# MathThyMod/GP_emu_UQSA

Measured on AMD Instinct MI355X. Metric: log-marginal-likelihood evals/sec at n=16384 d=10 fp64; 1/2/4/8 GPU, higher is better.
Workload: dtype f64

## Files before the change

gp_emu_uqsa_amd/csrc/gpemu.hip:

```cpp
#include <hip/hip_runtime.h>

#include <algorithm>
#include <array>
#include <atomic>
#include <map>
#include <cmath>
#include <cstdio>
#include <cstdlib>
#include <cstring>
#include <limits>
#include <string>
#include <vector>

#include "../../include/gpemu.h"
#include "gpemu_kernels.hpp"
#include "gpemu_gemm_sched.hpp"
#include "gpemu_small.hpp"
#include "gpemu_tiny.hpp"
#include "gpemu_snb.hpp"
#include "gpemu_ozaki.hpp"
#include "gpemu_pivchol.hpp"
#include "gpemu_imse.hpp"
#include "gpemu_postgrad.hpp"
#include "gpemu_postmean.hpp"
// ... 13 lines not shown
enum AdhocSlot {
  ADHOC_POST_V = ADHOC_DESC_BASE + 0,
  ADHOC_COV = ADHOC_DESC_BASE + 1,
  ADHOC_NOISE = ADHOC_DESC_BASE + 3,
  ADHOC_PIVCHOL = ADHOC_DESC_BASE + 4,
  ADHOC_POST_U = ADHOC_DESC_BASE + 5,
  ADHOC_IMSE = ADHOC_DESC_BASE + 7,
  ADHOC_TEST = ADHOC_DESC_BASE + 8,
  ADHOC_BENCH = ADHOC_DESC_BASE + 16,
};

struct Plan {
  long long n_pad = 0;
  const double* a_ptr = nullptr;
  const double* b_ptr = nullptr;
  std::vector<int> fused, fused_aug;
  std::vector<int> trtri;
  std::vector<std::vector<std::array<int, 3>>> tri_pairs;
  int lauum = -1;
  bool aug = false;
  std::vector<int> grp, grp_aug;
  int split_h = 0, aug_mid = -1;
  std::vector<int> sfused, sfused_aug, sgrp, sgrp_aug;
  bool sides = false;
  std::vector<std::array<int, 4>> trtri_side;
  std::vector<GemmLaunch> launches;
  std::vector<GemmProb> probs;
  std::vector<unsigned> tiles;
};

constexpr int FACT_FLAG_INTS = 6;

constexpr int OZ_CHOL_MIN = 8192;


struct Fact {
  long long n_pad = 0;
  int NB = 0;
  double* A = nullptr;
  double* B = nullptr;
  size_t cap = 0;
  double* logdet = nullptr;
  int* flags = nullptr;
  int* tflags = nullptr;
  bool aug = false;
  double* Faug = nullptr;
  double* part = nullptr;
  int* tcnt = nullptr;
  bool xdone[2] = {false, false};
  int xh = 0;
  int x11 = 0;
  bool t_ahead = false;
  void xclear(int h = 0) { xdone[0] = xdone[1] = t_ahead = false; x11 = 0; xh = h; }
  int desc_base = 0;
  Plan plan;
};
// ... 53 lines not shown
  double onel_tag = 0.0;
  int oz_on = 1, oz_nmod = OZ_MAXMOD;
  int oz_min_np = 6144;
  int oz_np2 = 0, oz_list_len = 0;
  long long oz_npad = 0;
  OzConst oz_c{};
  int8_t* dozp = nullptr;
  int8_t* dozr = nullptr;
  int* dozx = nullptr;
  unsigned* dozl = nullptr;
  double* dozt = nullptr;
  hipEvent_t ev_oz = nullptr;
  std::vector<OzTriPair> oz_tri;
  int oz_tri_min = 8192;
  double oz_lauum_ops = 0.0;
  int oz_chol = 1, oz_chol_min = OZ_CHOL_MIN;
  int tri_ahead_on = 1;
  hipEvent_t ev_l11 = nullptr, ev_schur = nullptr;
  OzTriPair oz_chol_q{};
  long long oz_chol_loff = 0;
  int oz_chol_llen = 0;
  double oz_chol_ops = 0.0;
  bool oz_chol_ready = false;
  bool oz_l21_valid = false;
  std::vector<hipEvent_t> oev;
  size_t oev_used = 0;
  double oz_ms = 0.0, oz_launches = 0.0, oz_ops = 0.0, oz_flops64 = 0.0;
  int dbg_skip_wait = -1;
  size_t small_cap = 0;

  double* hpin = nullptr;
  size_t hpin_cap = 0;

  float* dX32 = nullptr;
  size_t x32_cap = 0;
  bool x32_valid = false;
  float* dK32 = nullptr;
  size_t k32_cap = 0;
  hipEvent_t ev_pipe[2] = {nullptr, nullptr};
  int8_t* dpxp = nullptr;
  int* dpxe = nullptr;
  int8_t* dpkp = nullptr;
  int* dpke = nullptr;
  int8_t* dpres = nullptr;
  unsigned* dpl = nullptr;
  size_t pxp_cap = 0, pxe_cap = 0, pkp_cap = 0, pke_cap = 0, pres_cap = 0, pl_cap = 0;
// ... 237 lines not shown
  }
  return GPE_OK;
}

void add_launch(Plan& pl, GemmKind kind, const std::vector<GemmProb>& probs, double flops,
                const std::vector<unsigned>* order = nullptr) {
  GemmLaunch L = begin_launch(kind, pl.probs, flops);
  bool listable = probs.size() < 256;
  for (const GemmProb& p : probs) {
    push_prob(L, pl.probs, p, true);
    listable = listable && p.mt <= 4096 && p.nt <= 4096 && p.ksplit <= 1;
  }
  if (order) {
    set_list(L, pl.tiles, *order);
  } else if (listable) {
    const std::vector<unsigned> tl = order_tiles(probs);
    if ((int)tl.size() == L.tiles) set_list(L, pl.tiles, tl);
  }
  pl.launches.push_back(L);
}

bool oz_use(const gpe_ctx* c);
int oz_chol_split(const gpe_ctx* c, const Fact& F);

std::atomic<int> g_inflight[64];

struct InflightGuard {
  int dev;
  explicit InflightGuard(int d) : dev(d & 63) { g_inflight[dev].fetch_add(1); }
  ~InflightGuard() { g_inflight[dev].fetch_sub(1); }
};

struct AdhocGemm { GemmKind kind; GemmProb p; };
int adhoc_gemm(gpe_ctx* c, AdhocSlot slot, const std::vector<AdhocGemm>& g, GemmLaunch* out = nullptr,
               bool standalone = false) {
  std::vector<GemmProb> d;
  std::vector<GemmLaunch> launches;
  for (const AdhocGemm& e : g) {
    GemmLaunch L = begin_launch(e.kind, d);
    push_prob(L, d, e.p, standalone);
    L.first += slot;
    launches.push_back(L);
  }
  if (standalone)
    HIPCHK(c, hipMemcpy(c->dprobs + slot, d.data(), d.size() * sizeof(GemmProb), hipMemcpyHostToDevice));
  else
// ... 424 lines not shown
        for (const GemmProb& q : wb) { tb += prob_tiles(q); kb = std::max(kb, q.K); }
        for (int sd = 0; sd < 2; ++sd) {
          std::vector<GemmProb> pa, pb;
          double fa = 0.0, fb = 0.0;
          for (const auto& pr : trtri_side_pairs(pl.tri_pairs[lv], h, sd)) tri_pair(pr, pa, pb, fa, fb);
          if (pa.empty()) continue;
          split_k(pa, F.part, F.tcnt, ta, ka);
          split_k(pb, F.part, F.tcnt, tb, kb);
          side[2 * sd] = (int)pl.launches.size();
          add_launch(pl, GEMM_AK, pa, fa);
          side[2 * sd + 1] = (int)pl.launches.size();
          add_launch(pl, GEMM_PLAIN, pb, fb);
        }
        pl.trtri_side.push_back(side);
      }
      pl.sides = true;
      if ((int)pl.probs.size() > limit) {
        pl.launches.resize(nl1);
        pl.probs.resize(np1);
        pl.tiles.resize(nt1);
        pl.sides = false;
      }
    }
  }
  if ((int)pl.probs.size() > limit) return fail(c, GPE_ERR_UNSUPPORTED, "GEMM schedule too large");
  for (auto& L : pl.launches) L.first += F.desc_base;
  HIPCHK(c, hipMemcpy(c->dprobs + F.desc_base, pl.probs.data(), pl.probs.size() * sizeof(GemmProb),
                      hipMemcpyHostToDevice));
  const size_t half = pl.tiles.size() + 1;
  const size_t need = 2 * half;
  const bool regrow = need > c->tiles_cap;
  CHK(grow_buf(c, &c->dtiles, &c->tiles_cap, need));
  if (regrow) {
    Fact& other = (&F == &c->tr) ? c->aux : c->tr;
    other.plan = Plan();
  }
  const size_t base = (F.desc_base == 0) ? 0 : c->tiles_cap / 2;
  if (pl.tiles.size() > c->tiles_cap / 2) return fail(c, GPE_ERR_STATE, "tile list overflow");
  for (auto& L : pl.launches)
    if (L.list >= 0) L.list += (long long)base;
  if (!pl.tiles.empty())
    HIPCHK(c, hipMemcpy(c->dtiles + base, pl.tiles.data(), pl.tiles.size() * sizeof(unsigned),
                        hipMemcpyHostToDevice));
  return GPE_OK;
}

// ... 54 lines not shown
  if (kernel_alt(kernel)) {
    *coff = 1.0;
    *cdiag = predict ? 1.0 + nu * nu : 1.0;
  } else {
    *coff = 1.0 - nu;
    *cdiag = predict ? 1.0 : 1.0 - nu;
  }
}

int kbuild(gpe_ctx* c, int kernel, double nu, double s2, double rscale) {
  PairArgs a;
  a.xr = c->dXw; a.xc = c->dXw; a.out = c->tr.A; a.ld = c->n_pad;
  a.d = c->d; a.nr_valid = (int)c->n; a.nc_valid = (int)c->n;
  a.mt = c->NB; a.nt = c->NB; a.mode = 1 | 2;
  double coff, cdiag;
  kernel_consts(kernel, nu, true, &coff, &cdiag);
  a.s2 = s2; a.coff = coff; a.cdiag = cdiag;
  a.rscale = rscale; a.r = (c->has_r && rscale != 0.0) ? c->dr : nullptr;
  a.fam = kernel_fam(kernel);
  return launch_pairs(c, a, c->NB * (c->NB + 1) / 2);
}

int oz_prepare(gpe_ctx* c, Fact& F);
int chol_schur(gpe_ctx* c, Fact& F, hipStream_t st, bool with_aug);
int trtri(gpe_ctx* c, Fact& F, bool ozaki = false, bool ahead = false);

int potrf(gpe_ctx* c, Fact& F, bool with_aug = false, bool split = false, bool ahead = false) {
  CHK(build_plan(c, F));
  const int hs = split ? F.plan.split_h : 0;
  if (hs) CHK(oz_prepare(c, F));
  const Plan& pl = F.plan;
  if (hs != (split ? pl.split_h : 0)) return fail(c, GPE_ERR_STATE, "internal error: split plan changed");
  const int NB = F.NB;
  HIPCHK(c, hipMemsetAsync(F.flags, 0, FACT_FLAG_INTS * (size_t)NB * sizeof(int), c->stream));
  const bool wa = with_aug && pl.aug;
  const bool tri_ahead = hs && ahead && pl.sides && c->tri_ahead_on && c->chol_prio;
  F.xclear(tri_ahead ? hs : 0);
  const bool grp = c->potrf_group &&
                   (c->potrf_mode == 1 || (c->potrf_mode == 0 && g_inflight[c->device & 63].load() <= 1));
  const std::vector<int>& fidx = hs ? (grp ? (wa ? pl.sgrp_aug : pl.sgrp) : (wa ? pl.sfused_aug : pl.sfused))
                                    : (grp ? (wa ? pl.grp_aug : pl.grp) : (wa ? pl.fused_aug : pl.fused));
  if (c->chol_prio) {
    HIPCHK(c, hipEventRecord(c->ev_fork, c->stream));
    HIPCHK(c, hipStreamWaitEvent(c->stream2, c->ev_fork, 0));
    for (int t = 0; t < NB; ++t) {
      if (hs && t == hs) {
        if (tri_ahead) HIPCHK(c, hipEventRecord(c->ev_l11, c->stream2));
        CHK(chol_schur(c, F, c->stream2, wa));
        if (tri_ahead) {
          HIPCHK(c, hipEventRecord(c->ev_schur, c->stream2));
          CHK(trtri(c, F, true, true));
        }
      }
      if (fidx[t] >= 0) CHK(launch_gemm_range(c, pl.launches[fidx[t]], c->stream2));
    }
    HIPCHK(c, hipEventRecord(c->ev_join, c->stream2));
    HIPCHK(c, hipStreamWaitEvent(c->stream, c->ev_join, 0));
    return GPE_OK;
  }
#ifdef GEMM_TTRACE
  if (const char* es = std::getenv("GPEMU_DEBUG_STOP_STEP")) {
    const int stop = std::atoi(es);
    for (int t = 0; t <= stop && t < NB; ++t)
      if (fidx[t] >= 0) CHK(launch_gemm_range(c, pl.launches[fidx[t]]));
    HIPCHK(c, hipStreamSynchronize(c->stream));
    return fail(c, GPE_ERR_STATE, "debug stop after Cholesky launch " + std::to_string(stop));
  }
#endif
  for (int t = 0; t < NB; ++t) {
    if (hs && t == hs) CHK(chol_schur(c, F, c->stream, wa));
    if (fidx[t] >= 0) CHK(launch_gemm_range(c, pl.launches[fidx[t]]));
  }
  return GPE_OK;
}

void ev_rec(gpe_ctx* c, int i);

int lauum(gpe_ctx* c, Fact& F) {
  CHK(build_plan(c, F));
  return launch_gemm_range(c, F.plan.launches[F.plan.lauum]);
}

int ensure_xdiag(gpe_ctx* c, Fact& F, int side = -1) {
  const bool want0 = side != 1 && !F.xdone[0], want1 = side != 0 && !F.xdone[1];
  const int a = want0 ? 0 : F.xh, b = want1 ? F.NB : F.xh;
  if (b > a) {
    const long long off = (long long)a * TILE * (F.n_pad + 1);
    hipLaunchKernelGGL(k_xasm, dim3(b - a), dim3(256), DB_LDS_DOUBLES * sizeof(double), c->stream, F.A + off, F.B + off,
                       (long long)F.n_pad);
    HIPCHK(c, hipGetLastError());
  }
  F.xdone[0] = F.xdone[0] || want0;
  F.xdone[1] = F.xdone[1] || want1;
// ... 206 lines not shown
int z_from_factor(gpe_ctx* c);
int trsv_lower(gpe_ctx* c, Fact& F, const double* R, long long ldr, int P, double* Y, long long ldy);

int factor_and_invert(gpe_ctx* c, int kernel, const double* delta, double nu, double s2,
                      double rscale, bool invert = true, bool objective = false) {
  c->linv_valid = false;
  c->oz_l21_valid = false;
  HIPCHK(c, hipStreamSynchronize(c->stream2));
  HIPCHK(c, hipMemsetAsync(c->dinfo, 0, sizeof(int), c->stream));
  CHK(build_plan(c, c->tr));
  ev_rec(c, 0);
  CHK(scale_training(c, delta));
  CHK(kbuild(c, kernel, nu, s2, rscale));
  const int P = c->q + 1;
  c->zaug_valid = !invert && c->tr.plan.aug && P <= TILE;
  if (c->zaug_valid) {
    const long long tot = c->n_pad * TILE;
    hipLaunchKernelGGL(k_aug_init, dim3((unsigned)((tot + 255) / 256)), dim3(256), 0, c->stream, c->dF,
                       c->n_pad, P, c->n_pad, c->tr.Faug);
    HIPCHK(c, hipGetLastError());
  }
  ev_rec(c, 1);
  CHK(build_plan(c, c->tr));
  CHK(potrf(c, c->tr, c->zaug_valid, objective && (invert || c->oz_chol >= 2), objective && invert));
  if (kernel_fam(kernel) != FAM_GAUSS) {
    double coff, cdiag;
    kernel_consts(kernel, nu, true, &coff, &cdiag);
    const double floor_rel = 4.0 * (double)c->n_pad * std::numeric_limits<double>::epsilon();
    const double* r = (c->has_r && rscale != 0.0) ? c->dr : nullptr;
    hipLaunchKernelGGL(k_pivot_floor, dim3((unsigned)((c->n + 255) / 256)), dim3(256), 0, c->stream, c->tr.A,
                       c->n_pad, (int)c->n, floor_rel, s2 * cdiag, r, rscale, c->dinfo);
    HIPCHK(c, hipGetLastError());
  }
  ev_rec(c, 2);
  if (invert) {
    CHK(trtri(c, c->tr, true));
    c->linv_valid = true;
  }
  CHK(z_from_factor(c));
  ev_rec(c, 3);
  return GPE_OK;
}

int z_from_factor(gpe_ctx* c) {
  const int P = c->q + 1;
  const long long np = c->n_pad;
  if (c->zaug_valid) {
// ... 20 lines not shown
  CHK(ensure_xdiag(c, F));
  for (int c0 = 0; c0 < P; c0 += TS_PM) {
    const int pc = std::min(TS_PM, P - c0);
    HIPCHK(c, hipMemsetAsync(F.tflags, 0, 2 * sizeof(int), c->stream));
    hipLaunchKernelGGL(k_trsv_lower, dim3(F.NB), dim3(512), 0, c->stream, F.A, (long long)F.n_pad, F.B,
                       R + (long long)c0 * ldr, ldr, Y + (long long)c0 * ldy, ldy, pc, F.tflags, F.tflags + 1,
                       c->dinfo);
    HIPCHK(c, hipGetLastError());
  }
  return GPE_OK;
}

constexpr int OZ_MIN_NP = 6144, OZ_POST_MIN_NP = 4096, OZ_MAX_NP = 65536, OZ_POST_MAX_NP = 32768;
static_assert(OZ_MAX_NP % OZ_T == 0 && OZ_MAX_NP <= OZ_MAX_K && OZ_POST_MAX_NP <= OZ_MAX_K, "int8 sums too long");
bool oz_use(const gpe_ctx* c) { return c->oz_on && c->n_pad >= c->oz_min_np && c->n_pad <= OZ_MAX_NP; }

int oz_chol_split(const gpe_ctx* c, const Fact& F) {
  if (!c->oz_chol || !oz_use(c) || F.n_pad != c->n_pad || F.NB < 2) return 0;
  int h = 1;
  while (2 * h < F.NB) h *= 2;
  return (F.NB - h) * TILE >= c->oz_chol_min ? h : 0;
}

bool oz_tri_level(const gpe_ctx* c, const std::vector<std::array<int, 3>>& prs) {
  return oz_use(c) && !prs.empty() && (prs[0][1] - prs[0][0]) * TILE >= c->oz_tri_min;
}

int oz_prepare(gpe_ctx* c, Fact& F) {
  const int np2 = (int)(((c->n_pad + OZ_T - 1) / OZ_T) * OZ_T);
  if (c->n_pad == c->oz_npad && np2 == c->oz_np2 && c->oz_c.nmod == c->oz_nmod) return GPE_OK;
  c->oz_np2 = 0;
  c->oz_npad = 0;
  c->oz_chol_ready = false;
  c->oz_l21_valid = false;
  CHK(build_plan(c, F));
  const int N = c->oz_nmod;
  size_t planes = (size_t)oz_plane_bytes(np2) * N;
  size_t resid = (size_t)oz_lauum_shape(np2).res_bytes() * N;
  size_t scratch = 0, nex = (size_t)np2;
  std::vector<unsigned> all = oz_lauum_shape(np2).list();
  c->oz_list_len = (int)all.size();
  c->oz_lauum_ops = oz_lauum_shape(np2).ops(N);
  c->oz_tri.clear();
  for (const auto& prs : F.plan.tri_pairs) {
    if (!oz_tri_level(c, prs)) continue;
    for (const auto& pr : prs) {
      const OzTriPair q = oz_tri_pair_plan(pr[0], pr[1], pr[2], N, all);
      planes = std::max(planes, q.planes_bytes(N));
      resid = std::max(resid, q.resid_bytes(N));
      scratch = std::max(scratch, (size_t)q.Pa * q.Pb);
      nex = std::max(nex, (size_t)(q.Pa + q.Pb));
      c->oz_tri.push_back(q);
    }
  }
  if (const int hs = (&F == &c->tr) ? F.plan.split_h : 0) {
    const OzTriPair* have = nullptr;
    for (const OzTriPair& q : c->oz_tri)
      if (q.t0 == 0 && q.h == hs && q.t1 == F.NB) have = &q;
    const OzTriPair q = have ? *have : oz_tri_pair_plan(0, hs, F.NB, N, all);
    const std::vector<unsigned> ls = q.shape_schur().list();
    c->oz_chol_q = q;
    c->oz_chol_loff = (long long)all.size();
    c->oz_chol_llen = (int)ls.size();
    all.insert(all.end(), ls.begin(), ls.end());
    c->oz_chol_ops = q.shape_schur().ops(N);
    planes = std::max(planes, (size_t)N * q.Pb * q.Pa);
    resid = std::max(resid, (size_t)q.shape_schur().res_bytes() * N);
    nex = std::max(nex, (size_t)q.Pb);
    c->oz_chol_ready = true;
  }
  CHK(dalloc(c, &c->dozp, planes));
  CHK(dalloc(c, &c->dozr, resid));
  CHK(dalloc(c, &c->dozx, nex));
  CHK(dalloc(c, &c->dozt, scratch));
  CHK(dalloc(c, &c->dozl, all.size()));
  HIPCHK(c, hipMemcpy(c->dozl, all.data(), all.size() * sizeof(unsigned), hipMemcpyHostToDevice));
  c->oz_c = oz_consts(N, np2);
  c->oz_np2 = np2;
  c->oz_npad = c->n_pad;
  return GPE_OK;
}

int oz_gemm_crt(gpe_ctx* c, const OzConst& k, const OzProduct& p, double ops, double flops64,
                hipStream_t st = nullptr) {
  if (!st) st = c->stream;
  hipEvent_t e0 = nullptr, e1 = nullptr;
  if (c->prof) {
    while (c->oev_used + 2 > c->oev.size()) {
      hipEvent_t e;
      HIPCHK(c, hipEventCreate(&e));
      c->oev.push_back(e);
    }
    e0 = c->oev[c->oev_used];
    e1 = c->oev[c->oev_used + 1];
  }
  HIPCHK(c, oz_product_launch(st, k, p, e0, e1));
  if (c->prof) {
    c->oev_used += 2;
    c->oz_launches += 1.0;
    c->oz_ops += ops;
    c->oz_flops64 += flops64;
  }
  return GPE_OK;
}

int chol_schur(gpe_ctx* c, Fact& F, hipStream_t st, bool with_aug) {
  const Plan& pl = F.plan;
  const OzTriPair& q = c->oz_chol_q;
  if (!c->oz_chol_ready || q.h != pl.split_h) return fail(c, GPE_ERR_STATE, "internal error: split Cholesky without an int8 plan");
  if (with_aug) CHK(launch_gemm_range(c, pl.launches[pl.aug_mid], st));
  const long long ld = F.n_pad;
  oz_operand(st, c->oz_c, q.l21(F.A + (long long)q.h * TILE, ld), q.Pb, q.Pa, c->dozx, c->dozp);
  HIPCHK(c, hipGetLastError());
  const OzShape s = q.shape_schur();
  const OzOpnd l21{c->dozp, (long long)q.Pb * q.Pa, q.Pa, 0};
  CHK(oz_gemm_crt(c, c->oz_c,
                  OzProduct{s, l21, l21, c->dozl + c->oz_chol_loff, c->oz_chol_llen, c->dozr, s.res_bytes(),
                            OzOut{c->dozx, c->dozx, F.A + (long long)q.h * TILE * (ld + 1), ld, q.Rb, q.Rb, 1, -1.0, 1}},
                  c->oz_chol_ops, (double)q.Rb * q.Rb * q.Ra, st));
  c->oz_l21_valid = true;
  return GPE_OK;
}

int lauum_ozaki(gpe_ctx* c, Fact& F) {
  CHK(oz_prepare(c, F));
  const int np = (int)F.n_pad, np2 = c->oz_np2;
  c->oz_l21_valid = false;
  oz_operand_packed(c->stream, c->oz_c, F.B, (long long)F.n_pad, np, np2, c->dozx, c->dozp);
  const OzShape s = oz_lauum_shape(np2);
  const OzOpnd x{c->dozp, oz_plane_bytes(np2), 0, np2};
// ... 119 lines not shown
  {
    const char* ea = std::getenv("GPEMU_AUG");
    c->tr.aug = !(ea && std::string(ea) == "0");
  }
  {
    const char* e2 = std::getenv("GPEMU_POTRF");
    if (e2) {
      const std::string m(e2);
      c->potrf_group = m == "group" || m == "auto";
      c->potrf_mode = m == "group" ? 1 : (m == "auto" ? 0 : 2);
    }
    if (const char* eg = std::getenv("GPEMU_GROUP_P0")) c->grp_p0 = std::max(1, std::atoi(eg));
    if (const char* eg = std::getenv("GPEMU_GROUP_STRIDE")) c->grp_stride = std::max(0, std::atoi(eg));
    if (const char* ep = std::getenv("GPEMU_CHOL_PRIO")) c->chol_prio = std::atoi(ep) != 0;
    if (const char* et = std::getenv("GPEMU_TINY")) c->tiny = std::atoi(et) != 0;
    if (const char* ed = std::getenv("GPEMU_DEBUG_SKIP_WAIT")) c->dbg_skip_wait = std::atoi(ed);
    if (const char* em = std::getenv("GPEMU_MEAN_CHUNK")) c->mean_chunk = std::max(1, std::atoi(em) / 128) * 128LL;
    if (const char* eo = std::getenv("GPEMU_OZAKI")) c->oz_on = std::atoi(eo) != 0;
    if (const char* en = std::getenv("GPEMU_OZAKI_MIN_NP")) c->oz_min_np = std::max(512, std::atoi(en));
    if (const char* em = std::getenv("GPEMU_OZAKI_MODULI")) c->oz_nmod = std::max(8, std::min(OZ_MAXMOD, std::atoi(em)));
    if (const char* et = std::getenv("GPEMU_OZAKI_TRI_MIN")) c->oz_tri_min = std::max(512, std::atoi(et));
    if (const char* ec = std::getenv("GPEMU_OZAKI_CHOL")) c->oz_chol = std::max(0, std::min(3, std::atoi(ec)));
    if (const char* ec = std::getenv("GPEMU_OZAKI_CHOL_MIN")) c->oz_chol_min = std::max(256, std::atoi(ec));
    if (const char* ea = std::getenv("GPEMU_TRTRI_AHEAD")) c->tri_ahead_on = std::atoi(ea) != 0;
    if (const char* es = std::getenv("GPEMU_POTRF_SB")) {
      c->potrf_sb = std::max(1, std::min(8, std::atoi(es)));
      if (const char* colon = std::strchr(es, ':')) c->potrf_sb_min = std::max(0, std::atoi(colon + 1));
    }
    if (const char* e3 = std::getenv("GPEMU_POTRF_W")) {
      c->potrf_groups.clear();
      std::string spec(e3);
      size_t pos = 0;
      while (pos < spec.size()) {
        size_t end = spec.find(',', pos);
        if (end == std::string::npos) end = spec.size();
        const std::string item = spec.substr(pos, end - pos);
        const size_t colon = item.find(':');
        const int w = std::atoi(item.substr(0, colon).c_str());
        const int lim = colon == std::string::npos ? 0 : std::atoi(item.substr(colon + 1).c_str());
        if (w >= 1 && w <= 8) c->potrf_groups.push_back({w, lim});
        pos = end + 1;
      }
    }
  }
  if (hipSetDevice(device) != hipSuccess || hipStreamCreateWithFlags(&c->stream, hipStreamNonBlocking) != hipSuccess ||
      !create_priority_stream(&c->stream2) ||
// ... 2123 lines not shown
  const auto bad = [&](const char* what) { return fail(c, GPE_ERR_ARG, std::string("gpe_test_oz_product: ") + what); };
  if (p.nmod < 6 || p.nmod > OZ_MAXMOD) return bad("nmod outside [6, 16]");
  if (res_out && (p.res_mod < 0 || p.res_mod >= p.nmod)) return bad("res_mod is not a modulus number");
  if (a.R < 1 || a.R > (1 << 20)) return bad("bad operand rows");
  const int Pa = (a.R + OZ_T - 1) / OZ_T * OZ_T;
  int Pb = Pa;
  if (p.packed) {
    if (a.R % TILE || (a.offset & 1) || (a.ld & 1) || a.ld < a.R || !oz_test_extent(a, 1, 1) ||
        (long long)(a.R - 1) * a.ld + a.R > a.len - a.offset)
      return bad("packed: X is R x R, R a multiple of 128, ld >= R and offset even, inside src");
    p.K = Pa; p.kbeg = 1; p.kend = 0; p.kdiv = 1; p.ti0 = 0; p.tri = 1; p.lower128 = 1;
    p.rows = p.cols = a.R;
    b = nullptr;
  } else {
    if (p.K < OZ_SK || p.K % OZ_SK || p.K > OZ_MAX_K) return bad("K is not a multiple of 64 in [64, 2^17 - 128]");
    if (a.mask < 0 || a.mask > 2 || a.Kv > p.K || !oz_test_extent(a, a.R, a.Kv)) return bad("operand A outside its source");
    if (b) {
      if (b->R < 1 || b->R > (1 << 20) || b->mask < 0 || b->mask > 2 || b->Kv > p.K || !oz_test_extent(*b, b->R, b->Kv))
        return bad("operand B outside its source");
      Pb = (b->R + OZ_T - 1) / OZ_T * OZ_T;
    }
    if (p.kbeg < 0 || p.kbeg > 3 || p.kend < 0 || p.kend > 1 || p.kdiv < 1) return bad("bad kbeg / kend / kdiv");
    if (p.ti0 < 0 || p.ti0 >= Pa / OZ_T) return bad("ti0 past the last tile row");
    if (p.tri && Pb < Pa) return bad("tri: B has fewer tile rows than A");
  }
  if (p.rows <= OZ_T * p.ti0 || p.rows > Pa || p.cols < 1 || p.cols > Pb) return bad("rows / cols outside the product");
  if (!C || p.ldc < 1 || p.c_len < 1 || (long long)(p.rows - 1 - OZ_T * p.ti0) + (long long)(p.cols - 1) * p.ldc >= p.c_len)
    return bad("C too small for rows x cols at ldc");
  const int K = p.K, ti0 = p.ti0, nti = Pa / OZ_T - ti0, ntj = Pb / OZ_T;
  const OzConst k = oz_consts(p.nmod, K);
  const OzShape s{nti, p.tri ? 0 : ntj, ti0, p.tri ? 1 : 0, K, p.kbeg, p.kend, p.kdiv};
  OzTestBufs d;
  hipStream_t st = c->stream;
  OzOpnd oa, ob;
  if (p.packed) {
    CHK(dalloc(c, &d.sa, (size_t)a.len));
    CHK(dalloc(c, &d.exa, (size_t)Pa));
    CHK(dalloc(c, &d.pa, (size_t)k.nmod * oz_plane_bytes(Pa)));
    HIPCHK(c, hipMemcpy(d.sa, a.src, (size_t)a.len * sizeof(double), hipMemcpyHostToDevice));
    oz_operand_packed(st, k, d.sa + a.offset, (long long)a.ld, a.R, Pa, d.exa, d.pa);
    HIPCHK(c, hipGetLastError());
    oa = ob = OzOpnd{d.pa, oz_plane_bytes(Pa), 0, Pa};
  } else {
    CHK(oz_test_operand(c, a, k, Pa, K, &d.sa, &d.exa, &d.pa));
    oa = ob = OzOpnd{d.pa, (long long)Pa * K, K, 0};
    if (b) {
      CHK(oz_test_operand(c, *b, k, Pb, K, &d.sb, &d.exb, &d.pb));
      ob = OzOpnd{d.pb, (long long)Pb * K, K, 0};
    }
  }
  const std::vector<unsigned> list = s.list();
  const long long rb = s.res_bytes();
  CHK(dalloc(c, &d.list, list.size()));
  CHK(dalloc(c, &d.res, (size_t)k.nmod * rb));
  CHK(dalloc(c, &d.C, (size_t)p.c_len));
  HIPCHK(c, hipMemcpy(d.list, list.data(), list.size() * sizeof(unsigned), hipMemcpyHostToDevice));
  HIPCHK(c, hipMemcpy(d.C, C, (size_t)p.c_len * sizeof(double), hipMemcpyHostToDevice));
  HIPCHK(c, hipMemsetAsync(d.res, 0, (size_t)k.nmod * rb, st));
  const OzOut out{d.exa, b ? d.exb : d.exa, d.C, (long long)p.ldc, p.rows, p.cols, p.lower128 ? 1 : 0, p.alpha, p.acc ? 1 : 0};
  CHK(oz_gemm_crt(c, k, OzProduct{s, oa, ob, d.list, (int)list.size(), d.res, rb, out}, 0.0, 0.0));
  HIPCHK(c, hipStreamSynchronize(st));
  HIPCHK(c, hipMemcpy(C, d.C, (size_t)p.c_len * sizeof(double), hipMemcpyDeviceToHost));
  if (exa_out) HIPCHK(c, hipMemcpy(exa_out, d.exa, (size_t)Pa * sizeof(int), hipMemcpyDeviceToHost));
  if (exb_out) HIPCHK(c, hipMemcpy(exb_out, b ? d.exb : d.exa, (size_t)Pb * sizeof(int), hipMemcpyDeviceToHost));
  if (res_out) {
    std::vector<int8_t> h((size_t)rb);
    HIPCHK(c, hipMemcpy(h.data(), d.res + (long long)p.res_mod * rb, (size_t)rb, hipMemcpyDeviceToHost));
    std::memset(res_out, 0, (size_t)nti * OZ_T * Pb);
    const auto tile_of = [&](long long ti, long long tj) { return p.tri ? ti * (ti + 1) / 2 + tj : ti * ntj + tj; };
    for (const unsigned ent : list) {
      if (ent == 0xffffffffu) continue;
      const int ti = (int)(ent >> 16), tj = (int)(ent & 0xffffu);
      const int8_t* t = h.data() + (tile_of(ti, tj) - tile_of(ti0, 0)) * (OZ_T * OZ_T);
      for (int u = 0; u < OZ_T * OZ_T / 16; ++u) {
        const int wave = u >> 10, blk = (u >> 6) & 15, lane = u & 63;
        const long long gm = OZ_T * (ti - ti0) + (wave >> 1) * 128 + 32 * (blk >> 2) + (lane & 31);
        const long long gn0 = OZ_T * tj + (wave & 1) * 128 + 32 * (blk & 3) + 4 * (lane >> 5);
        for (int q = 0; q < 16; ++q) res_out[gm * Pb + gn0 + (q & 3) + 8 * (q >> 2)] = t[(long long)u * 16 + q];
      }
    }
  }
  return GPE_OK;
}

int gpe_test_oz_product(gpe_ctx* c, const gpe_oz_operand* a, const gpe_oz_operand* b, const gpe_oz_params* p, double* C,
                        int32_t* exa_out, int32_t* exb_out, int8_t* res_out) {
  if (!c) return GPE_ERR_ARG;
  if (!a || !p) return fail(c, GPE_ERR_ARG, "gpe_test_oz_product: NULL operand or parameters");
  HIPCHK(c, hipSetDevice(c->device));
  const bool prof = c->prof;
  c->prof = false;
  const int rc = oz_test_product(c, *a, b, *p, C, exa_out, exb_out, res_out);
  c->prof = prof;
  return rc;
}

// ... 190 lines not shown
```

gp_emu_uqsa_amd/csrc/gpemu_ozaki.hpp:

```cpp
#pragma once
#include <algorithm>
#include <array>
#include <cmath>
#include <cstdlib>
#include <cstring>
#include <type_traits>
#include <utility>
#include <vector>

namespace gpe {

constexpr int OZ_T = 256;
constexpr int OZ_SK = 64;
constexpr int OZ_NBUF = 4;
constexpr int OZ_OPND = OZ_T * OZ_SK;
constexpr int OZ_LDS = OZ_NBUF * 2 * OZ_OPND;
constexpr int OZ_MAXMOD = 16;
constexpr int OZ_MAX_K = (1 << 17) - 128;

struct OzConst {
  int m[OZ_MAXMOD];
  int c16[OZ_MAXMOD];
  float inv[OZ_MAXMOD];
  double rhi[OZ_MAXMOD];
// ... 87 lines not shown
  long long ld;
  int np2;
};
__device__ __forceinline__ const int8_t* oz_tile_rows(const OzOpnd& o, int t, int k, long long& ld) {
  if (o.ld == 0) {
    ld = o.np2 - OZ_T * t;
    return o.p + oz_panel_off(t, o.np2) + (k - OZ_T * t);
  }
  ld = o.ld;
  return o.p + (long long)OZ_T * t * o.ld + k;
}

struct OzGemm {
  OzOpnd a, b;
  const unsigned* list;
  int list_len;
  int K, kbeg, kend;
  int tri, ntj;
  int8_t* res;
  long long res_bytes;
  int kdiv = 1;
  int ti0 = 0;
};
__device__ __forceinline__ long long oz_res_tile(int tri, int ntj, int ti, int tj) {
  return tri ? (long long)ti * (ti + 1) / 2 + tj : (long long)ti * ntj + tj;
}
__host__ __device__ __forceinline__ void oz_k_range(int kbeg, int kend, int kdiv, int K, int ti, int tj, int& kb, int& ke) {
  kb = kbeg == 1 ? OZ_T * ti : (kbeg == 2 ? OZ_T * tj : (kbeg == 3 ? 128 * ((2 * ti) / kdiv) : 0));
  ke = kend == 1 ? (K < OZ_T * (ti + 1) ? K : OZ_T * (ti + 1)) : K;
}

__device__ __forceinline__ void oz_vmwait_stages(int stages) {
  static_assert(OZ_NBUF <= 5, "one case per stage that can be in flight");
  if (stages >= 4) oz_vmwait<32>();
  else if (stages == 3) oz_vmwait<24>();
  else if (stages == 2) oz_vmwait<16>();
  else if (stages == 1) oz_vmwait<8>();
  else oz_vmwait<0>();
}

template <bool M256>
__device__ __forceinline__ void oz_store_residues(const oz_v16i (&acc)[4][4], int m, int c16, float inv, int8_t* out) {
#pragma clang fp contract(off)
  const int cm = c16 - 65536, nm = -m;
#pragma unroll
  for (int i = 0; i < 4; ++i)
#pragma unroll
    for (int j = 0; j < 4; ++j) {
// ... 143 lines not shown
                ((long long)(wave * 16) * 64 + lane) * 16;
  if (m == 256) oz_store_residues<true>(acc, m, 0, 0.0f, out);
  else oz_store_residues<false>(acc, m, cst.c16[l], cst.inv[l], out);
}

struct OzCrt {
  const int8_t* res;
  long long res_bytes;
  int tri, ntj;
  const int* exr;
  const int* exc;
  double* C;
  long long ldc;
  int rows, cols, lower128;
  double alpha;
  int ti0 = 0;
  int acc = 0;
};
static __global__ void __launch_bounds__(256) k_oz_crt(OzCrt g, OzConst cst) {
  const int t = (int)blockIdx.x >> 4;
  const int u = ((int)blockIdx.x & 15) * 256 + (int)threadIdx.x;
  int ti, tj;
  if (g.tri) {
    const int ta = t + g.ti0 * (g.ti0 + 1) / 2;
    ti = g.ti0;
    while ((ti + 1) * (ti + 2) / 2 <= ta) ++ti;
    tj = ta - ti * (ti + 1) / 2;
  } else {
    ti = g.ti0 + t / g.ntj;
    tj = t % g.ntj;
  }
  const int wave = u >> 10, blk = (u >> 6) & 15, lane = u & 63;
  const int i = blk >> 2, j = blk & 3;
  const int gm = OZ_T * ti + (wave >> 1) * 128 + 32 * i + (lane & 31);
  const int gn0 = OZ_T * tj + (wave & 1) * 128 + 32 * j + 4 * (lane >> 5);
  if (gm >= g.rows || gn0 >= g.cols) return;
  double shi[16], slo[16];
#pragma unroll
  for (int r = 0; r < 16; ++r) shi[r] = slo[r] = 0.0;
  const int8_t* src = g.res + (long long)t * (OZ_T * OZ_T) + (long long)u * 16;
  for (int l = 0; l < cst.nmod; ++l) {
    const oz_v4i w = *reinterpret_cast<const oz_v4i*>(src + (long long)l * g.res_bytes);
    const double rh = cst.rhi[l], rl = cst.rlo[l];
#pragma unroll
    for (int r = 0; r < 16; ++r) {
      const double cv = (double)(int)(int8_t)((unsigned)w[r >> 2] >> (8 * (r & 3)));
      shi[r] = fma(cv, rh, shi[r]);
      slo[r] = fma(cv, rl, slo[r]);
    }
  }
// ... 181 lines not shown
    k.rlo[l] = std::ldexp((double)R / (double)m, -41);
  }
  return k;
}

template <class W>
std::vector<unsigned> oz_list(int nti, int ntj, bool lower, W work, int ti0 = 0) {
  static const std::pair<int, int> blk = [] {
    int r = 8, c = 4;
    if (const char* e = std::getenv("GPEMU_OZ_BLOCK")) {
      const int rr = std::atoi(e);
      const char* x = std::strchr(e, 'x');
      if (rr > 0 && x && std::atoi(x + 1) > 0) { r = rr; c = std::atoi(x + 1); }
    }
    return std::make_pair(r, c);
  }();
  const int OZ_BR = blk.first, OZ_BC = blk.second;
  struct Blk { double w; std::vector<unsigned> t; };
  std::vector<Blk> blks;
  for (int r0 = ti0; r0 < ti0 + nti; r0 += OZ_BR)
    for (int c0 = 0; c0 < ntj && (!lower || c0 <= r0 + OZ_BR - 1); c0 += OZ_BC) {
      Blk b{0.0, {}};
      for (int ti = r0; ti < std::min(ti0 + nti, r0 + OZ_BR); ++ti)
        for (int tj = c0; tj < std::min(lower ? ti + 1 : ntj, c0 + OZ_BC); ++tj) {
          b.t.push_back(((unsigned)ti << 16) | (unsigned)tj);
          b.w += work(ti, tj);
        }
      if (!b.t.empty()) blks.push_back(std::move(b));
    }
  std::stable_sort(blks.begin(), blks.end(), [](const Blk& x, const Blk& y) { return x.w / x.t.size() > y.w / y.t.size(); });
  std::vector<std::vector<unsigned>> bins(8);
  std::vector<double> load(8, 0.0);
  for (const Blk& b : blks) {
    const int x = (int)(std::min_element(load.begin(), load.end()) - load.begin());
    load[x] += b.w;
    bins[x].insert(bins[x].end(), b.t.begin(), b.t.end());
  }
  size_t longest = 0;
  for (auto& b : bins) longest = std::max(longest, b.size());
  std::vector<unsigned> list(8 * longest, 0xffffffffu);
  for (int x = 0; x < 8; ++x)
    for (size_t q = 0; q < bins[x].size(); ++q) list[8 * q + x] = bins[x][q];
  return list;
}


struct OzSrc {
// ... 14 lines not shown
}
inline void oz_operand_split(hipStream_t st, const OzConst& k, const OzSrc& o, int P, int Kp, const int* ex, int8_t* planes) {
  if (o.trans)
    hipLaunchKernelGGL(k_oz_split_rect<true>, dim3(P / 64, Kp / 64), dim3(256), 0, st, o.src, o.ld, o.R, o.Kv, o.mask, ex,
                       planes, (long long)P * Kp, (long long)Kp, Kp, k);
  else
    hipLaunchKernelGGL(k_oz_split_rect<false>, dim3(P, (Kp + 2047) / 2048), dim3(256), 0, st, o.src, o.ld, o.R, o.Kv,
                       o.mask, ex, planes, (long long)P * Kp, (long long)Kp, Kp, k);
}
inline void oz_operand(hipStream_t st, const OzConst& k, const OzSrc& o, int P, int Kp, int* ex, int8_t* planes) {
  oz_operand_exp(st, k, o, P, ex);
  oz_operand_split(st, k, o, P, Kp, ex, planes);
}
inline void oz_operand_packed(hipStream_t st, const OzConst& k, const double* X, long long ldx, int np, int np2, int* ex,
                              int8_t* planes) {
  hipLaunchKernelGGL(k_oz_colexp, dim3((np2 + 3) / 4), dim3(256), 0, st, X, ldx, np, np2, k.beta, ex);
  hipLaunchKernelGGL(k_oz_split, dim3(np2, (np2 + 256 * OZ_SPLIT_ROWS - 1) / (256 * OZ_SPLIT_ROWS)), dim3(256), 0, st, X,
                     ldx, np, np2, ex, planes, oz_plane_bytes(np2), k);
}

struct OzShape {
  int nti, ntj, ti0, tri, K, kbeg, kend, kdiv;
  static OzShape lower(int nti, int ti0, int K, int kbeg, int kdiv = 1) { return {nti, 0, ti0, 1, K, kbeg, 0, kdiv}; }
  static OzShape rect(int nti, int ntj, int K, int kbeg, int kend) { return {nti, ntj, 0, 0, K, kbeg, kend, 1}; }
  int klen(int ti, int tj) const {
    int kb, ke;
    oz_k_range(kbeg, kend, kdiv, K, ti, tj, kb, ke);
    return std::max(0, ke - kb);
  }
  std::vector<unsigned> list() const {
    return oz_list(nti, tri ? ti0 + nti : ntj, tri != 0, [&](int ti, int tj) { return (double)klen(ti, tj); }, ti0);
  }
  long long tiles() const {
    const long long t1 = ti0 + nti;
    return tri ? t1 * (t1 + 1) / 2 - (long long)ti0 * (ti0 + 1) / 2 : (long long)nti * ntj;
  }
  long long res_bytes() const { return tiles() * OZ_T * OZ_T; }
  double ops(int N) const {
    double s = 0.0;
    for (int ti = ti0; ti < ti0 + nti; ++ti)
      for (int tj = 0; tj < (tri ? ti + 1 : ntj); ++tj) s += klen(ti, tj);
    return 2.0 * OZ_T * OZ_T * s * N;
  }
};

inline OzShape oz_lauum_shape(int np2) { return OzShape::lower(np2 / OZ_T, 0, np2, 1); }
inline OzShape oz_slab_shape(int a0, int a1, int Kp, int P) {
  return OzShape::lower((a1 + 1) / 2 - a0 / 2, a0 / 2, Kp, 3, P);
}

struct OzOut {
  const int* exr;
  const int* exc;
  double* C;
  long long ldc;
  int rows, cols, lower128;
  double alpha;
  int acc = 0;
};
struct OzProduct {
  OzShape s;
  OzOpnd a, b;
  const unsigned* list;
  int list_len;
  int8_t* res;
  long long res_bytes;
  OzOut out;
};
inline hipError_t oz_product_launch(hipStream_t st, const OzConst& k, const OzProduct& p, hipEvent_t e0 = nullptr,
                                    hipEvent_t e1 = nullptr) {
  const OzShape& s = p.s;
  const int ntj = s.tri ? 0 : s.ntj;
  const OzGemm g{p.a, p.b, p.list, p.list_len, s.K, s.kbeg, s.kend, s.tri, ntj, p.res, p.res_bytes, s.kdiv, s.ti0};
  const OzOut& o = p.out;
  const OzCrt r{p.res, p.res_bytes, s.tri, ntj, o.exr, o.exc, o.C, o.ldc, o.rows, o.cols, o.lower128, o.alpha, s.ti0, o.acc};
  hipError_t e;
  if (e0 && (e = hipEventRecord(e0, st)) != hipSuccess) return e;
  hipLaunchKernelGGL(k_oz_gemm, dim3((unsigned)(k.nmod * g.list_len)), dim3(256), OZ_LDS, st, g, k);
  if (e1 && (e = hipEventRecord(e1, st)) != hipSuccess) return e;
  hipLaunchKernelGGL(k_oz_crt, dim3((unsigned)(s.tiles() * 16)), dim3(256), 0, st, r, k);
  return hipGetLastError();
}

inline std::vector<std::array<int, 3>> trtri_level_pairs(int NB, int s) {
  std::vector<std::array<int, 3>> prs;
  for (int t0 = 0; t0 < NB; t0 += s) {
    const int h = t0 + s / 2;
    if (h >= NB) continue;
    prs.push_back({t0, h, std::min(t0 + s, NB)});
  }
  return prs;
}

inline std::vector<std::array<int, 3>> trtri_side_pairs(const std::vector<std::array<int, 3>>& prs, int hs, int side) {
  std::vector<std::array<int, 3>> out;
// ... 13 lines not shown
  size_t planes_bytes(int N) const { return (size_t)N * Pa * (Pa + Pb); }
  size_t resid_bytes(int N) const { return (size_t)N * shape_a().res_bytes(); }
  OzSrc l21(const double* L21, long long ld) const { return {L21, ld, Rb, Ra, 0, true}; }
};
inline OzTriPair oz_tri_pair_plan(int t0, int h, int t1, int N, std::vector<unsigned>& lists) {
  OzTriPair q;
  q.t0 = t0; q.h = h; q.t1 = t1;
  q.Ra = (h - t0) * TILE;
  q.Rb = (t1 - h) * TILE;
  q.Pa = (q.Ra + OZ_T - 1) / OZ_T * OZ_T;
  q.Pb = (q.Rb + OZ_T - 1) / OZ_T * OZ_T;
  const std::vector<unsigned> la = q.shape_a().list(), lb = q.shape_b().list();
  q.ops_a = q.shape_a().ops(N);
  q.ops_b = q.shape_b().ops(N);
  q.la_off = (long long)lists.size();
  q.la_len = (int)la.size();
  lists.insert(lists.end(), la.begin(), la.end());
  q.lb_off = (long long)lists.size();
  q.lb_len = (int)lb.size();
  lists.insert(lists.end(), lb.begin(), lb.end());
  return q;
}

template <class GC>
void oz_tri_pair_launches(hipStream_t st, const OzConst& k, const OzTriPair& q, const unsigned* lists, const double* L21,
                          const double* X11, const double* X22, double* X21, long long ld, double* T, int8_t* planes,
                          int8_t* res, int* ex, bool l21_done, GC gc, int part = 0) {
  int* exA = ex;
  int* exB = ex + q.Pb;
  int8_t* PA = planes;
  const long long rb = q.shape_a().res_bytes();
  if (part != 2) {
    const long long pA = (long long)q.Pb * q.Pa, pB = (long long)q.Pa * q.Pa;
    int8_t* PB = planes + (size_t)k.nmod * pA;
    if (!l21_done) oz_operand(st, k, q.l21(L21, ld), q.Pb, q.Pa, exA, PA);
    oz_operand(st, k, OzSrc{X11, ld, q.Ra, q.Ra, 1, false}, q.Pa, q.Pa, exB, PB);
    gc(OzProduct{q.shape_a(), OzOpnd{PA, pA, q.Pa, 0}, OzOpnd{PB, pB, q.Pa, 0}, lists + q.la_off, q.la_len, res, rb,
                 OzOut{exA, exB, T, (long long)q.Pb, q.Rb, q.Ra, 0, 1.0}},
       q.ops_a, (double)q.Ra * q.Ra * q.Rb);
  }
  if (part != 1) {
    const long long pA = (long long)q.Pb * q.Pb, pB = (long long)q.Pa * q.Pb;
    int8_t* PB = planes + (size_t)k.nmod * pA;
    const OzSrc x22{X22, ld, q.Rb, q.Rb, 2, true}, t{T, (long long)q.Pb, q.Ra, q.Rb, 0, false};
    oz_operand_exp(st, k, x22, q.Pb, exA);
    oz_operand_exp(st, k, t, q.Pa, exB);
// ... 10 lines not shown
```

Measured before the change: 19.46.

## Add nested int8 Ozaki split point inside the first Cholesky half

Adds a second split point at half of the existing Cholesky split. The trailing Schur update from the first q block columns onto the region past q is done as one int8 Ozaki emulated GEMM, with a capped-lower-triangle tile shape, instead of the fp64 per-panel GEMM launches. The Ozaki tile indexing, list building and test harness are generalised to support lower triangles capped at a column count. The aim is to move more of the O(n^3) update work onto faster int8 matrix units, at the cost of extra operand splitting, larger scratch buffers and more emulation error exposure.

```diff
diff --git a/gp_emu_uqsa_amd/csrc/gpemu.hip b/gp_emu_uqsa_amd/csrc/gpemu.hip
--- a/gp_emu_uqsa_amd/csrc/gpemu.hip
+++ b/gp_emu_uqsa_amd/csrc/gpemu.hip
@@ -59,6 +59,8 @@
   std::vector<int> grp, grp_aug;
   int split_h = 0, aug_mid = -1;
   std::vector<int> sfused, sfused_aug, sgrp, sgrp_aug;
+  int split_q = 0, aug_q = -1;
+  std::vector<int> nfused, nfused_aug, ngrp, ngrp_aug;
   bool sides = false;
   std::vector<std::array<int, 4>> trtri_side;
   std::vector<GemmLaunch> launches;
@@ -69,6 +71,7 @@
 constexpr int FACT_FLAG_INTS = 6;
 
 constexpr int OZ_CHOL_MIN = 8192;
+constexpr int OZ_CHOL_NEST_MIN = 12288;
 
 
 struct Fact {
@@ -168,6 +171,12 @@
   int oz_chol_llen = 0;
   double oz_chol_ops = 0.0;
   bool oz_chol_ready = false;
+  int oz_nest = 1, oz_nest_min = OZ_CHOL_NEST_MIN;
+  OzCholNest oz_nest_q{};
+  long long oz_nest_loff = 0;
+  int oz_nest_llen = 0;
+  double oz_nest_ops = 0.0;
+  bool oz_nest_ready = false;
   bool oz_l21_valid = false;
   std::vector<hipEvent_t> oev;
   size_t oev_used = 0;
@@ -451,6 +460,7 @@
 
 bool oz_use(const gpe_ctx* c);
 int oz_chol_split(const gpe_ctx* c, const Fact& F);
+int oz_chol_nest_split(const gpe_ctx* c, const Fact& F, int h);
 
 std::atomic<int> g_inflight[64];
 
@@ -921,6 +931,33 @@
         pl.sides = false;
       }
     }
+    if (const int q = pl.split_h ? oz_chol_nest_split(c, F, h) : 0) {
+      const size_t nl2 = pl.launches.size(), np2 = pl.probs.size(), nt2 = pl.tiles.size();
+      pl.nfused.assign(NB, -1);
+      pl.nfused_aug.assign(NB, -1);
+      if (c->potrf_group) {
+        pl.ngrp.assign(NB, -1);
+        if (pl.aug) pl.ngrp_aug.assign(NB, -1);
+      }
+      const std::array<std::vector<int>*, 4> nx = {&pl.nfused, &pl.nfused_aug, &pl.ngrp, &pl.ngrp_aug};
+      CHK(sweep(0, q, NB, nx));
+      CHK(sweep(q, h - q, NB - q, nx));
+      for (int v = 0; v < 4; ++v)
+        for (int t = h; t < NB && !nx[v]->empty(); ++t) (*nx[v])[t] = (*ix[v])[t];
+      if (pl.aug) {
+        pl.aug_q = (int)pl.launches.size();
+        add_launch(pl, GEMM_PLAIN, {mkprob(F.Faug, TILE, tile(A, q, 0), ld, F.Faug + (long long)q * TILE * TILE, TILE, 1, h - q,
+                                  q * TILE, 0, -1.0, 1.0)}, 0.0);
+      }
+      pl.split_q = q;
+      if ((int)pl.probs.size() > limit) {
+        pl.launches.resize(nl2);
+        pl.probs.resize(np2);
+        pl.tiles.resize(nt2);
+        pl.split_q = 0;
+        pl.aug_q = -1;
+      }
+    }
   }
   if ((int)pl.probs.size() > limit) return fail(c, GPE_ERR_UNSUPPORTED, "GEMM schedule too large");
   for (auto& L : pl.launches) L.first += F.desc_base;
@@ -1021,15 +1058,16 @@
 }
 
 int oz_prepare(gpe_ctx* c, Fact& F);
-int chol_schur(gpe_ctx* c, Fact& F, hipStream_t st, bool with_aug);
+int chol_schur(gpe_ctx* c, Fact& F, hipStream_t st, bool with_aug, int at);
 int trtri(gpe_ctx* c, Fact& F, bool ozaki = false, bool ahead = false);
 
-int potrf(gpe_ctx* c, Fact& F, bool with_aug = false, bool split = false, bool ahead = false) {
+int potrf(gpe_ctx* c, Fact& F, bool with_aug = false, bool split = false, bool ahead = false, bool nest = false) {
   CHK(build_plan(c, F));
   const int hs = split ? F.plan.split_h : 0;
   if (hs) CHK(oz_prepare(c, F));
   const Plan& pl = F.plan;
   if (hs != (split ? pl.split_h : 0)) return fail(c, GPE_ERR_STATE, "internal error: split plan changed");
+  const int qs = (hs && nest) ? pl.split_q : 0;
   const int NB = F.NB;
   HIPCHK(c, hipMemsetAsync(F.flags, 0, FACT_FLAG_INTS * (size_t)NB * sizeof(int), c->stream));
   const bool wa = with_aug && pl.aug;
@@ -1037,15 +1075,17 @@
   F.xclear(tri_ahead ? hs : 0);
   const bool grp = c->potrf_group &&
                    (c->potrf_mode == 1 || (c->potrf_mode == 0 && g_inflight[c->device & 63].load() <= 1));
-  const std::vector<int>& fidx = hs ? (grp ? (wa ? pl.sgrp_aug : pl.sgrp) : (wa ? pl.sfused_aug : pl.sfused))
-                                    : (grp ? (wa ? pl.grp_aug : pl.grp) : (wa ? pl.fused_aug : pl.fused));
+  const std::vector<int>& fidx = qs ? (grp ? (wa ? pl.ngrp_aug : pl.ngrp) : (wa ? pl.nfused_aug : pl.nfused))
+                                 : hs ? (grp ? (wa ? pl.sgrp_aug : pl.sgrp) : (wa ? pl.sfused_aug : pl.sfused))
+                                      : (grp ? (wa ? pl.grp_aug : pl.grp) : (wa ? pl.fused_aug : pl.fused));
   if (c->chol_prio) {
     HIPCHK(c, hipEventRecord(c->ev_fork, c->stream));
     HIPCHK(c, hipStreamWaitEvent(c->stream2, c->ev_fork, 0));
     for (int t = 0; t < NB; ++t) {
+      if (qs && t == qs) CHK(chol_schur(c, F, c->stream2, wa, qs));
       if (hs && t == hs) {
         if (tri_ahead) HIPCHK(c, hipEventRecord(c->ev_l11, c->stream2));
-        CHK(chol_schur(c, F, c->stream2, wa));
+        CHK(chol_schur(c, F, c->stream2, wa, hs));
         if (tri_ahead) {
           HIPCHK(c, hipEventRecord(c->ev_schur, c->stream2));
           CHK(trtri(c, F, true, true));
@@ -1067,7 +1107,8 @@
   }
 #endif
   for (int t = 0; t < NB; ++t) {
-    if (hs && t == hs) CHK(chol_schur(c, F, c->stream, wa));
+    if (qs && t == qs) CHK(chol_schur(c, F, c->stream, wa, qs));
+    if (hs && t == hs) CHK(chol_schur(c, F, c->stream, wa, hs));
     if (fidx[t] >= 0) CHK(launch_gemm_range(c, pl.launches[fidx[t]]));
   }
   return GPE_OK;
@@ -1320,7 +1361,8 @@
   }
   ev_rec(c, 1);
   CHK(build_plan(c, c->tr));
-  CHK(potrf(c, c->tr, c->zaug_valid, objective && (invert || c->oz_chol >= 2), objective && invert));
+  CHK(potrf(c, c->tr, c->zaug_valid, objective && (invert || c->oz_chol >= 2), objective && invert,
+            objective && (invert || c->oz_chol == 3)));
   if (kernel_fam(kernel) != FAM_GAUSS) {
     double coff, cdiag;
     kernel_consts(kernel, nu, true, &coff, &cdiag);
@@ -1387,6 +1429,11 @@
   return (F.NB - h) * TILE >= c->oz_chol_min ? h : 0;
 }
 
+int oz_chol_nest_split(const gpe_ctx* c, const Fact& F, int h) {
+  if (!c->oz_nest || h < 4 || (h / 2) % 2) return 0;
+  return (F.NB - h / 2) * TILE >= c->oz_nest_min ? h / 2 : 0;
+}
+
 bool oz_tri_level(const gpe_ctx* c, const std::vector<std::array<int, 3>>& prs) {
   return oz_use(c) && !prs.empty() && (prs[0][1] - prs[0][0]) * TILE >= c->oz_tri_min;
 }
@@ -1397,6 +1444,7 @@
   c->oz_np2 = 0;
   c->oz_npad = 0;
   c->oz_chol_ready = false;
+  c->oz_nest_ready = false;
   c->oz_l21_valid = false;
   CHK(build_plan(c, F));
   const int N = c->oz_nmod;
@@ -1433,6 +1481,19 @@
     resid = std::max(resid, (size_t)q.shape_schur().res_bytes() * N);
     nex = std::max(nex, (size_t)q.Pb);
     c->oz_chol_ready = true;
+    if (const int qs = F.plan.split_q) {
+      const OzCholNest nq = oz_chol_nest_plan(qs, hs, F.NB);
+      const std::vector<unsigned> ln = nq.shape().list();
+      c->oz_nest_q = nq;
+      c->oz_nest_loff = (long long)all.size();
+      c->oz_nest_llen = (int)ln.size();
+      all.insert(all.end(), ln.begin(), ln.end());
+      c->oz_nest_ops = nq.shape().ops(N);
+      planes = std::max(planes, nq.planes_bytes(N));
+      resid = std::max(resid, nq.resid_bytes(N));
+      nex = std::max(nex, (size_t)nq.Pb);
+      c->oz_nest_ready = true;
+    }
   }
   CHK(dalloc(c, &c->dozp, planes));
   CHK(dalloc(c, &c->dozr, resid));
@@ -1469,8 +1530,24 @@
   return GPE_OK;
 }
 
-int chol_schur(gpe_ctx* c, Fact& F, hipStream_t st, bool with_aug) {
+int chol_schur(gpe_ctx* c, Fact& F, hipStream_t st, bool with_aug, int at) {
   const Plan& pl = F.plan;
+  if (at != pl.split_h) {
+    const OzCholNest& n = c->oz_nest_q;
+    if (!c->oz_nest_ready || at != pl.split_q || n.q != at || n.h != pl.split_h)
+      return fail(c, GPE_ERR_STATE, "internal error: nested split Cholesky without an int8 plan");
+    if (with_aug) CHK(launch_gemm_range(c, pl.launches[pl.aug_q], st));
+    const long long ld = F.n_pad;
+    c->oz_l21_valid = false;
+    oz_operand(st, c->oz_c, n.src(F.A + (long long)n.q * TILE, ld), n.Pb, n.K, c->dozx, c->dozp);
+    HIPCHK(c, hipGetLastError());
+    const OzShape s = n.shape();
+    const OzOpnd l{c->dozp, (long long)n.Pb * n.K, n.K, 0};
+    return oz_gemm_crt(c, c->oz_c,
+                       OzProduct{s, l, l, c->dozl + c->oz_nest_loff, c->oz_nest_llen, c->dozr, s.res_bytes(),
+                                 OzOut{c->dozx, c->dozx, F.A + (long long)n.q * TILE * (ld + 1), ld, n.Rb, n.cols, 1, -1.0, 1}},
+                       c->oz_nest_ops, (double)n.cols * (2.0 * n.Rb - n.cols) * n.K, st);
+  }
   const OzTriPair& q = c->oz_chol_q;
   if (!c->oz_chol_ready || q.h != pl.split_h) return fail(c, GPE_ERR_STATE, "internal error: split Cholesky without an int8 plan");
   if (with_aug) CHK(launch_gemm_range(c, pl.launches[pl.aug_mid], st));
@@ -1636,6 +1713,8 @@
     if (const char* et = std::getenv("GPEMU_OZAKI_TRI_MIN")) c->oz_tri_min = std::max(512, std::atoi(et));
     if (const char* ec = std::getenv("GPEMU_OZAKI_CHOL")) c->oz_chol = std::max(0, std::min(3, std::atoi(ec)));
     if (const char* ec = std::getenv("GPEMU_OZAKI_CHOL_MIN")) c->oz_chol_min = std::max(256, std::atoi(ec));
+    if (const char* ec = std::getenv("GPEMU_OZAKI_CHOL_NEST")) c->oz_nest = std::atoi(ec) != 0;
+    if (const char* ec = std::getenv("GPEMU_OZAKI_CHOL_NEST_MIN")) c->oz_nest_min = std::max(256, std::atoi(ec));
     if (const char* ea = std::getenv("GPEMU_TRTRI_AHEAD")) c->tri_ahead_on = std::atoi(ea) != 0;
     if (const char* es = std::getenv("GPEMU_POTRF_SB")) {
       c->potrf_sb = std::max(1, std::min(8, std::atoi(es)));
@@ -3805,14 +3884,14 @@
     }
     if (p.kbeg < 0 || p.kbeg > 3 || p.kend < 0 || p.kend > 1 || p.kdiv < 1) return bad("bad kbeg / kend / kdiv");
     if (p.ti0 < 0 || p.ti0 >= Pa / OZ_T) return bad("ti0 past the last tile row");
-    if (p.tri && Pb < Pa) return bad("tri: B has fewer tile rows than A");
+    if (p.tri && Pb < Pa && p.ti0 != 0) return bad("tri: B has fewer tile rows than A and ti0 > 0");
   }
   if (p.rows <= OZ_T * p.ti0 || p.rows > Pa || p.cols < 1 || p.cols > Pb) return bad("rows / cols outside the product");
   if (!C || p.ldc < 1 || p.c_len < 1 || (long long)(p.rows - 1 - OZ_T * p.ti0) + (long long)(p.cols - 1) * p.ldc >= p.c_len)
     return bad("C too small for rows x cols at ldc");
   const int K = p.K, ti0 = p.ti0, nti = Pa / OZ_T - ti0, ntj = Pb / OZ_T;
   const OzConst k = oz_consts(p.nmod, K);
-  const OzShape s{nti, p.tri ? 0 : ntj, ti0, p.tri ? 1 : 0, K, p.kbeg, p.kend, p.kdiv};
+  const OzShape s{nti, p.tri ? (Pb < Pa ? ntj : 0) : ntj, ti0, p.tri ? 1 : 0, K, p.kbeg, p.kend, p.kdiv};
   OzTestBufs d;
   hipStream_t st = c->stream;
   OzOpnd oa, ob;
@@ -3850,11 +3929,10 @@
     std::vector<int8_t> h((size_t)rb);
     HIPCHK(c, hipMemcpy(h.data(), d.res + (long long)p.res_mod * rb, (size_t)rb, hipMemcpyDeviceToHost));
     std::memset(res_out, 0, (size_t)nti * OZ_T * Pb);
-    const auto tile_of = [&](long long ti, long long tj) { return p.tri ? ti * (ti + 1) / 2 + tj : ti * ntj + tj; };
     for (const unsigned ent : list) {
       if (ent == 0xffffffffu) continue;
       const int ti = (int)(ent >> 16), tj = (int)(ent & 0xffffu);
-      const int8_t* t = h.data() + (tile_of(ti, tj) - tile_of(ti0, 0)) * (OZ_T * OZ_T);
+      const int8_t* t = h.data() + s.res_tile(ti, tj) * (OZ_T * OZ_T);
       for (int u = 0; u < OZ_T * OZ_T / 16; ++u) {
         const int wave = u >> 10, blk = (u >> 6) & 15, lane = u & 63;
         const long long gm = OZ_T * (ti - ti0) + (wave >> 1) * 128 + 32 * (blk >> 2) + (lane & 31);
diff --git a/gp_emu_uqsa_amd/csrc/gpemu_ozaki.hpp b/gp_emu_uqsa_amd/csrc/gpemu_ozaki.hpp
--- a/gp_emu_uqsa_amd/csrc/gpemu_ozaki.hpp
+++ b/gp_emu_uqsa_amd/csrc/gpemu_ozaki.hpp
@@ -133,8 +133,10 @@
   int kdiv = 1;
   int ti0 = 0;
 };
-__device__ __forceinline__ long long oz_res_tile(int tri, int ntj, int ti, int tj) {
-  return tri ? (long long)ti * (ti + 1) / 2 + tj : (long long)ti * ntj + tj;
+__host__ __device__ __forceinline__ long long oz_res_tile(int tri, int ntj, int ti, int tj) {
+  if (!tri) return (long long)ti * ntj + tj;
+  if (ntj > 0 && ti >= ntj) return (long long)ntj * (ntj + 1) / 2 + (long long)(ti - ntj) * ntj + tj;
+  return (long long)ti * (ti + 1) / 2 + tj;
 }
 __host__ __device__ __forceinline__ void oz_k_range(int kbeg, int kend, int kdiv, int K, int ti, int tj, int& kb, int& ke) {
   kb = kbeg == 1 ? OZ_T * ti : (kbeg == 2 ? OZ_T * tj : (kbeg == 3 ? 128 * ((2 * ti) / kdiv) : 0));
@@ -324,10 +326,15 @@
   const int u = ((int)blockIdx.x & 15) * 256 + (int)threadIdx.x;
   int ti, tj;
   if (g.tri) {
-    const int ta = t + g.ti0 * (g.ti0 + 1) / 2;
-    ti = g.ti0;
-    while ((ti + 1) * (ti + 2) / 2 <= ta) ++ti;
-    tj = ta - ti * (ti + 1) / 2;
+    const int ta = t + (int)oz_res_tile(1, g.ntj, g.ti0, 0), cap = g.ntj * (g.ntj + 1) / 2;
+    if (g.ntj > 0 && ta >= cap) {
+      ti = g.ntj + (ta - cap) / g.ntj;
+      tj = (ta - cap) % g.ntj;
+    } else {
+      ti = g.ti0;
+      while ((ti + 1) * (ti + 2) / 2 <= ta) ++ti;
+      tj = ta - ti * (ti + 1) / 2;
+    }
   } else {
     ti = g.ti0 + t / g.ntj;
     tj = t % g.ntj;
@@ -555,7 +562,7 @@
     for (int c0 = 0; c0 < ntj && (!lower || c0 <= r0 + OZ_BR - 1); c0 += OZ_BC) {
       Blk b{0.0, {}};
       for (int ti = r0; ti < std::min(ti0 + nti, r0 + OZ_BR); ++ti)
-        for (int tj = c0; tj < std::min(lower ? ti + 1 : ntj, c0 + OZ_BC); ++tj) {
+        for (int tj = c0; tj < std::min(std::min(lower ? ti + 1 : ntj, ntj), c0 + OZ_BC); ++tj) {
           b.t.push_back(((unsigned)ti << 16) | (unsigned)tj);
           b.w += work(ti, tj);
         }
@@ -616,24 +623,24 @@
 struct OzShape {
   int nti, ntj, ti0, tri, K, kbeg, kend, kdiv;
   static OzShape lower(int nti, int ti0, int K, int kbeg, int kdiv = 1) { return {nti, 0, ti0, 1, K, kbeg, 0, kdiv}; }
+  static OzShape lower_capped(int nti, int cap, int K) { return {nti, cap < nti ? cap : 0, 0, 1, K, 0, 0, 1}; }
   static OzShape rect(int nti, int ntj, int K, int kbeg, int kend) { return {nti, ntj, 0, 0, K, kbeg, kend, 1}; }
+  int row_tiles(int ti) const { return tri ? (ntj > 0 ? std::min(ti + 1, ntj) : ti + 1) : ntj; }
   int klen(int ti, int tj) const {
     int kb, ke;
     oz_k_range(kbeg, kend, kdiv, K, ti, tj, kb, ke);
     return std::max(0, ke - kb);
   }
   std::vector<unsigned> list() const {
-    return oz_list(nti, tri ? ti0 + nti : ntj, tri != 0, [&](int ti, int tj) { return (double)klen(ti, tj); }, ti0);
-  }
-  long long tiles() const {
-    const long long t1 = ti0 + nti;
-    return tri ? t1 * (t1 + 1) / 2 - (long long)ti0 * (ti0 + 1) / 2 : (long long)nti * ntj;
-  }
+    return oz_list(nti, tri && ntj == 0 ? ti0 + nti : ntj, tri != 0, [&](int ti, int tj) { return (double)klen(ti, tj); }, ti0);
+  }
+  long long res_tile(int ti, int tj) const { return oz_res_tile(tri, ntj, ti, tj) - oz_res_tile(tri, ntj, ti0, 0); }
+  long long tiles() const { return tri ? oz_res_tile(1, ntj, ti0 + nti, 0) - oz_res_tile(1, ntj, ti0, 0) : (long long)nti * ntj; }
   long long res_bytes() const { return tiles() * OZ_T * OZ_T; }
   double ops(int N) const {
     double s = 0.0;
     for (int ti = ti0; ti < ti0 + nti; ++ti)
-      for (int tj = 0; tj < (tri ? ti + 1 : ntj); ++tj) s += klen(ti, tj);
+      for (int tj = 0; tj < row_tiles(ti); ++tj) s += klen(ti, tj);
     return 2.0 * OZ_T * OZ_T * s * N;
   }
 };
@@ -664,7 +671,7 @@
 inline hipError_t oz_product_launch(hipStream_t st, const OzConst& k, const OzProduct& p, hipEvent_t e0 = nullptr,
                                     hipEvent_t e1 = nullptr) {
   const OzShape& s = p.s;
-  const int ntj = s.tri ? 0 : s.ntj;
+  const int ntj = s.ntj;
   const OzGemm g{p.a, p.b, p.list, p.list_len, s.K, s.kbeg, s.kend, s.tri, ntj, p.res, p.res_bytes, s.kdiv, s.ti0};
   const OzOut& o = p.out;
   const OzCrt r{p.res, p.res_bytes, s.tri, ntj, o.exr, o.exc, o.C, o.ldc, o.rows, o.cols, o.lower128, o.alpha, s.ti0, o.acc};
@@ -724,6 +731,23 @@
   return q;
 }
 
+struct OzCholNest {
+  int q, h, NB, Rb, Pb, K, cols;
+  OzShape shape() const { return OzShape::lower_capped(Pb / OZ_T, (h - q) / 2, K); }
+  OzSrc src(const double* Lq0, long long ld) const { return {Lq0, ld, Rb, K, 0, true}; }
+  size_t planes_bytes(int N) const { return (size_t)N * Pb * K; }
+  size_t resid_bytes(int N) const { return (size_t)N * shape().res_bytes(); }
+};
+inline OzCholNest oz_chol_nest_plan(int q, int h, int NB) {
+  OzCholNest n;
+  n.q = q; n.h = h; n.NB = NB;
+  n.Rb = (NB - q) * TILE;
+  n.Pb = (n.Rb + OZ_T - 1) / OZ_T * OZ_T;
+  n.K = q * TILE;
+  n.cols = (h - q) * TILE;
+  return n;
+}
+
 template <class GC>
 void oz_tri_pair_launches(hipStream_t st, const OzConst& k, const OzTriPair& q, const unsigned* lists, const double* L21,
                           const double* X11, const double* X22, double* X21, long long ld, double* T, int8_t* planes,
```

New measurement: 19.75, median of 6. 1.01x the previous value.
